# VIS4ROB-lab/covins

Hardware: AMD Instinct MI355X
Metric: GBA iterations/sec, 5-agent EuRoC merged map (higher is better)
Workload: dtype f64

## Files before the change

covins_amd/backend.py:

```python
from __future__ import annotations

import ctypes as C
import os
import subprocess
from typing import Optional, Tuple

import numpy as np

from . import capi
from .capi import FlatProblem, Options, Result, dptr, iptr

_HERE = os.path.dirname(os.path.abspath(__file__))
_SO = os.path.join(_HERE, "libcovgpu.so")
if os.environ.get("COVGPU_LIBRARY"):
    _SO = os.environ["COVGPU_LIBRARY"]
_LIB: Optional[C.CDLL] = None


class CovGpuError(RuntimeError):
    pass


def build(force: bool = False) -> str:
    args = ["make", "-C", os.path.join(_HERE, "csrc"), "-j8"]
# ... 234 lines not shown
        f = np.ascontiguousarray(f, dtype=np.float64).reshape(-1, 4, 3)
        P = np.ascontiguousarray(P, dtype=np.float64).reshape(-1, 4, 3)
        n = f.shape[0]
        T = np.zeros((max(n, 1), 4, 7)); ns = np.zeros(max(n, 1), np.int32); ch = np.zeros(max(n, 1), np.int32)
        self._check(lib().covgpu_p3p_batch(self._h, n, dptr(f), dptr(P), dptr(T), iptr(ns), iptr(ch)))
        return T[:n], ns[:n], ch[:n]

    def set_profiling(self, on: bool):
        lib().covgpu_set_profiling(self._h, int(on))

    def profile(self) -> dict:
        out = np.zeros(16)
        lib().covgpu_get_profile2(self._h, dptr(out))
        return dict(build_ms=out[0], n_build=int(out[1]), factor_ms=out[2], n_factor=int(out[3]), syrk_ms=out[4],
                    n_syrk=int(out[5]), syrk_flops=out[6], offdiag_blocks=int(out[7]),
                    potrf_ms=out[8], n_potrf=int(out[9]), potrf_flops=out[10], plan_flops=out[11])

    def layout(self) -> dict:
        out = (C.c_int64 * 16)()
        lib().covgpu_get_layout(self._h, out)
        keys = ("shard_world", "shard_rank", "top_unknowns", "top_levels", "allreduce_kib", "stream_ordering", "dense_order", "covisible_pairs",
                "edge_pairs", "chains", "device_mib", "nd_fronts", "nd_levels", "nd_serial_panels", "nd_root_order", "nd_front_mib")
        return {k: int(out[i]) for i, k in enumerate(keys)}

    def residual_norms(self, prob, opt):
        out = np.zeros(prob.O); s = prob.as_struct()
        self._check(lib().covgpu_reprojection_residual_norms(self._h, C.byref(opt), C.byref(s), dptr(out)))
        return out

    def linearize_reprojection(self, prob, opt):
        O = prob.O
# ... 55 lines not shown
```

covins_amd/csrc/common.hpp:

```cpp
#pragma once
#include <hip/hip_runtime.h>
#include <atomic>
#include <cstdlib>
#include <stdint.h>

#include <map>
#include <unordered_map>
#include <utility>
#include <vector>

#include "../../include/covgpu.h"

namespace covgpu {

constexpr int kTile = 128;

struct DevProblem {
  int K, A, L, O, I, E, S;
  int D;
  int n;
  int npad;
  int N;
  int vi;
  int lm_group;
// ... 117 lines not shown
  return P.Sred + (size_t)(6 * pi + r) * P.npad + (6 * pj + c);
}

enum { SC_COST = 0, SC_JV2 = 1, SC_GG = 2, SC_GN2 = 3, SC_GDOT = 4, SC_GMAX = 5, SC_GS = 6, SC_SN2 = 7, SC_XN2 = 8,
       SC_VV = 9, SC_VG = 10, SC_NN = 11, SC_JA = 12, SC_JB = 13, SC_JC = 14,
       SC_COUNT = 16 };

struct CholAux;
inline bool first_use_on_device(std::atomic<unsigned long long>& seen) {
  int d = 0;
  if (hipGetDevice(&d) != hipSuccess || d < 0 || d > 63) return true;
  const unsigned long long bit = 1ull << d;
  return (seen.fetch_or(bit, std::memory_order_acq_rel) & bit) == 0;
}
struct DevSignal { long long* flag = nullptr; long long seq = 0; };
inline int env_int(const char* name, int fallback) {
  const char* e = getenv(name);
  return e != nullptr ? atoi(e) : fallback;
}
void launch_kobs_build(const DevProblem& P, int* pair_oa, int* pair_ob, size_t nent, hipStream_t st);
void launch_lm_lin(const DevProblem& P, double mu, hipStream_t st, DevSignal sig = DevSignal());
void launch_lm_build(const DevProblem& P, double mu, hipStream_t st, hipEvent_t pose_system_cleared = nullptr, hipStream_t side = nullptr,
                     hipEvent_t ev_lin = nullptr, hipEvent_t ev_kf = nullptr, CholAux* ax = nullptr);
void launch_lm_backsub(const DevProblem& P, const double* dp, double* out_all, hipStream_t st);
void launch_obs_jvp(const DevProblem& P, const double* v_all, hipStream_t st);
void launch_obs_cost(const DevProblem& P, const double* pose, const double* lm, hipStream_t st);
void launch_obs_linearize(const DevProblem& P, double* r, double* Jp, double* Jl, double* cost, hipStream_t st);
void launch_obs_norms(const DevProblem& P, double* norms, hipStream_t st);
void launch_lm_outliers(const DevProblem& P, double th, unsigned char* erase, int* left, unsigned long long* counts, hipStream_t st);

// ... 58 lines not shown
  long long* gate_flags = nullptr;
  int* gate_dead = nullptr;
  int* gate_dead_h = nullptr;
  std::unordered_map<hipEvent_t, int> gate_slot;
  std::map<std::pair<hipEvent_t, hipStream_t>, int> gate_slot_es;
  std::vector<long long> gate_seq;
  long long gate_counter = 0;
  double gate_timeout_s = 3.0;
  long gate_signals = 0, gate_waits = 0;
  void record(hipEvent_t e, hipStream_t s, int tag = 0);
  void wait(hipStream_t s, hipEvent_t e0, hipEvent_t e1 = nullptr, hipEvent_t e2 = nullptr, hipEvent_t e3 = nullptr);
  DevSignal publish_handle(hipEvent_t e, hipStream_t s, int tag = 0);
  void record_handle(DevSignal d, hipStream_t s);
  void sync(hipStream_t s, hipEvent_t r0, int tag0, hipEvent_t r1, int tag1, hipEvent_t w0 = nullptr, hipEvent_t w1 = nullptr, hipEvent_t w2 = nullptr,
            hipEvent_t w3 = nullptr);
  int gate_slot_of(hipEvent_t e, hipStream_t s);
  long long* gate_log = nullptr; int gate_log_n = 0;
  std::vector<int> gate_log_tag; std::vector<char> gate_log_kind; std::vector<int> gate_tag_of_slot;
  static constexpr int kGateLogMax = 16384;
  bool gate_failed() const { return gate_dead_h != nullptr && *(volatile int*)gate_dead_h != 0; }
  void gates_disable();
};
struct BwdXfer {
  const int* gidx = nullptr;
  const int *own_g = nullptr, *st_g = nullptr, *own_dims = nullptr, *st_dims = nullptr;
  double* x = nullptr;
  int first = 0;
};
struct DenseBatch {
  int n = 0; size_t sM = 0, sL = 0, sR = 0;
// ... 37 lines not shown
void launch_bwd_front(const double* S, int tI, int ntiles, int nchunk, double* y, const double* Linv, int nbt, size_t sL, size_t sR, hipStream_t st,
                      const long long* btab, const int* live, BwdXfer xf, int* cnt, double* scr);
void launch_bwd_pipe(const double* S, int tI, int ntiles, int nchunk, double* y, const double* Linv, int nbt, size_t sL, size_t sR, hipStream_t st,
                     const long long* btab, const int* live, BwdXfer xf, double* pipe, int* dead, int* dead_h, double timeout_s);
void launch_pipe_fill(double* buf, size_t n, hipStream_t st);
constexpr int kBwdTreeMax = 8;
constexpr int kPipeChunk = 128;
struct BwdTreeLevel {
  int nbt, T, nchunk, tI, first;
  double* y; size_t bsR; const double* Dinv; size_t bsL; const long long* btab; const int* live;
  size_t scr_off, xpub_off;
};
void launch_bwd_tree(const double* M, const BwdTreeLevel* lev, int nlev, BwdXfer xf, double* pipe, int* dead, int* dead_h, double timeout_s, hipStream_t st,
                     bool form64 = false);
unsigned long long pipe_empty_word();
void launch_trsm_sub(double* S, size_t ld, int t0, int w, int r0, int r1, const double* Linv, double* b, int npad, int nbt, size_t sM, size_t sL,
                     size_t sR, const int* live, int tI, hipStream_t st, bool chain = false, const long long* btab = nullptr, int nb = -1, const int* own = nullptr);
void launch_bwd_step_sub(const double* S, size_t ld, int p, const double* Linv_p, double* y, double* x, int ncol, int nblocks, int nbt, size_t sM,
                         size_t sL, size_t sR, hipStream_t st, const long long* btab = nullptr, const int* live = nullptr, int tI = 0,
                         BwdXfer xf = BwdXfer());

struct PgoHostPlan { std::vector<std::vector<int>> block_kf; std::vector<int> border_kf; };
bool pgo_plan_analyse(int K, int E, const int* ei, const int* ej, PgoHostPlan& out);
struct PgoPlan {
  bool active = false;
  int nblk = 0, nIpad = 0, ntot = 0;
  int nb = 0;
  int* idx = nullptr;
  double *M = nullptr, *rhs = nullptr, *Linv = nullptr;
  int* idx_b = nullptr;
  double *Sb = nullptr, *rhs_b = nullptr, *Linv_b = nullptr;
};
// ... 113 lines not shown
```

covins_amd/csrc/k_chol.hip:

```cpp
#include <algorithm>
#include <cstdio>
#include <cstdlib>
#include <mutex>

#include "common.hpp"
#include "dev_math.hpp"

namespace covgpu {
using namespace covdev;

typedef double v4f64 __attribute__((ext_vector_type(4)));

#ifdef COVGPU_PROBE
__device__ long long g_probe[8];
#define PROBE(i) do { if (threadIdx.x == 0) g_probe[i] = wall_clock64(); } while (0)
#define PROBE_ACC(i, t0) do { if (threadIdx.x == 0) g_probe[i] += wall_clock64() - (t0); } while (0)
#define PROBE_T0() wall_clock64()
#else
#define PROBE(i) do {} while (0)
#define PROBE_ACC(i, t0) do {} while (0)
#define PROBE_T0() 0
#endif

constexpr int KC = 16;
// ... 175 lines not shown
      }
    __syncthreads();
    if (tid < TSA) {
      double t = 0.0;
#pragma unroll
      for (int w2 = 0; w2 < WGC; ++w2) t += sp[w2 * TSA + tid];
      g.rhs[(size_t)batch * g.bsR + g.ra0 + ti * kTile + qr * TSA + tid] -= t;
    }
  }
}

template <int MODE>
__global__ __launch_bounds__(256, 2) void k_gemm_abt(GemmArgs g) { gemm_abt_body<MODE, kTile, kTile, KC, PFF>(g); }
template <int MODE, int TSA, int TSB>
__global__ __launch_bounds__(256, 2) void k_gemm_abt_q(GemmArgs g) { gemm_abt_body<MODE, TSA, TSB, KCQ, (MODE == MODE_SYRK_RECT ? PFR : PFQ)>(g); }

static hipStream_t make_side_stream(int priority) {
  hipStream_t s2 = nullptr;
  (void)hipStreamCreateWithPriority(&s2, hipStreamNonBlocking, priority);
  return s2;
}

void CholAux::init() {
  int lo = 0, hi = 0;
  (void)hipDeviceGetStreamPriorityRange(&lo, &hi);
  if (!head) (void)hipStreamCreateWithPriority(&head, hipStreamNonBlocking, hi);
  if (!mid) mid = make_side_stream(hi);
  if (!aux) aux = make_side_stream(lo);
  if (!ev_zero) (void)hipEventCreateWithFlags(&ev_zero, hipEventDisableTiming);
  if (!ev_lin) (void)hipEventCreateWithFlags(&ev_lin, hipEventDisableTiming);
  if (!ev_kf) (void)hipEventCreateWithFlags(&ev_kf, hipEventDisableTiming);
  if (!ev_fill) (void)hipEventCreateWithFlags(&ev_fill, hipEventDisableTiming);
  if (!ev_xb) (void)hipEventCreateWithFlags(&ev_xb, hipEventDisableTiming);
  if (!ev_xa) (void)hipEventCreateWithFlags(&ev_xa, hipEventDisableTiming);
  if (!bwd_cnt && hipMalloc((void**)&bwd_cnt, 65536 * sizeof(int)) == hipSuccess) (void)hipMemset(bwd_cnt, 0, 65536 * sizeof(int));
  if (!gate_dead && hipMalloc((void**)&gate_dead, sizeof(int)) == hipSuccess) (void)hipMemset(gate_dead, 0, sizeof(int));
  if (!gate_dead_h && hipHostMalloc((void**)&gate_dead_h, 4 * sizeof(int), hipHostMallocDefault) == hipSuccess) gate_dead_h[0] = gate_dead_h[1] = gate_dead_h[2] = gate_dead_h[3] = 0;
  if (const char* e = getenv("COVGPU_GATE_TIMEOUT_S")) gate_timeout_s = std::max(getenv("COVGPU_GATE_TIMEOUT_MIN") ? atof(getenv("COVGPU_GATE_TIMEOUT_MIN")) : 0.01, atof(e));
  if (!gate_flags && !gates_broken) {
    static const bool want = env_int("COVGPU_GATES", 1) != 0;
    if (want && gate_dead != nullptr && gate_dead_h != nullptr && hipMalloc((void**)&gate_flags, kGateSlots * sizeof(long long)) == hipSuccess) {
      (void)hipMemset(gate_flags, 0, kGateSlots * sizeof(long long));
      (void)hipDeviceSynchronize();
      gates_on = true;
      if (getenv("COVGPU_GATE_LOG") && hipMalloc((void**)&gate_log, 2 * (size_t)kGateLogMax * sizeof(long long)) != hipSuccess) gate_log = nullptr;
    } else gates_broken = true;
  }
}
__global__ void k_signal(long long* flag, long long seq, long long* log) {
  if (threadIdx.x == 0) {
    __hip_atomic_store(flag, seq, __ATOMIC_RELAXED, __HIP_MEMORY_SCOPE_AGENT);
    if (log) log[0] = wall_clock64();
  }
}
__global__ void k_signal2(DevSignal a, DevSignal b) {
  if (threadIdx.x != 0) return;
// ... 36 lines not shown
    if ((int)gate_seq.size() <= slot) gate_seq.resize(slot + 1, 0);
  }
  gate_slot[e] = slot;
  return slot;
}
void CholAux::record(hipEvent_t e, hipStream_t s, int tag) {
  if (!gates_on) { (void)hipEventRecord(e, s); return; }
  const int slot = gate_slot_of(e, s);
  if (slot < 0) { gate_slot.erase(e); (void)hipEventRecord(e, s); return; }
  gate_seq[slot] = ++gate_counter;
  long long* lg = nullptr;
  if ((int)gate_tag_of_slot.size() <= slot) gate_tag_of_slot.resize(slot + 1, 0);
  gate_tag_of_slot[slot] = tag;
  if (gate_log != nullptr && gate_log_n < kGateLogMax) { lg = gate_log + 2 * (size_t)gate_log_n++; gate_log_tag.push_back(tag); gate_log_kind.push_back('S'); }
  hipLaunchKernelGGL(k_signal, dim3(1), dim3(64), 0, s, gate_flags + slot, gate_seq[slot], lg);
  ++gate_signals;
}
DevSignal CholAux::publish_handle(hipEvent_t e, hipStream_t s, int tag) {
  DevSignal d;
  if (!gates_on) return d;
  const int slot = gate_slot_of(e, s);
  if (slot < 0) { gate_slot.erase(e); return d; }
  gate_seq[slot] = ++gate_counter;
  if ((int)gate_tag_of_slot.size() <= slot) gate_tag_of_slot.resize(slot + 1, 0);
  gate_tag_of_slot[slot] = tag;
  d.flag = gate_flags + slot; d.seq = gate_seq[slot];
  ++gate_signals;
  return d;
}
void CholAux::record_handle(DevSignal d, hipStream_t s) { if (d.flag != nullptr) hipLaunchKernelGGL(k_signal2, dim3(1), dim3(64), 0, s, d, DevSignal()); }
void CholAux::wait(hipStream_t s, hipEvent_t e0, hipEvent_t e1, hipEvent_t e2, hipEvent_t e3) { sync(s, nullptr, 0, nullptr, 0, e0, e1, e2, e3); }
void CholAux::sync(hipStream_t s, hipEvent_t r0, int tag0, hipEvent_t r1, int tag1, hipEvent_t e0, hipEvent_t e1, hipEvent_t e2, hipEvent_t e3) {
  hipEvent_t es[4] = {e0, e1, e2, e3};
  if (!gates_on) {
    if (r0 != nullptr) record(r0, s, tag0);
    if (r1 != nullptr) record(r1, s, tag1);
    for (hipEvent_t e : es) if (e != nullptr) (void)hipStreamWaitEvent(s, e, 0);
    return;
  }
  GateArgs g; g.n = 0; g.dead = gate_dead; g.dead_h = gate_dead_h; g.limit = (long long)(gate_timeout_s * 1e8); g.log = nullptr; g.np = 0; g.base = gate_flags;
  g.pf[0] = g.pf[1] = nullptr; g.ps[0] = g.ps[1] = 0;
  {
    hipEvent_t rs[2] = {r0, r1}; const int tags[2] = {tag0, tag1};
    for (int i = 0; i < 2; ++i) {
      if (rs[i] == nullptr) continue;
// ... 7 lines not shown
  }
  int first_tag = g.np > 0 ? -(r0 != nullptr ? tag0 : tag1) : 0;
  for (hipEvent_t e : es) {
    if (e == nullptr) continue;
    auto it = gate_slot.find(e);
    if (it == gate_slot.end()) { (void)hipStreamWaitEvent(s, e, 0); continue; }
    if (gate_seq[it->second] == 0) continue;
    if (g.n == 0 && g.np == 0 && it->second < (int)gate_tag_of_slot.size()) first_tag = gate_tag_of_slot[it->second];
    g.f[g.n] = gate_flags + it->second; g.s[g.n] = gate_seq[it->second]; ++g.n;
  }
  if (g.n == 0 && g.np == 0) return;
  if (gate_log != nullptr && gate_log_n < kGateLogMax) { g.log = gate_log + 2 * (size_t)gate_log_n++; gate_log_tag.push_back(first_tag); gate_log_kind.push_back('G'); }
  for (int i = g.n; i < 4; ++i) { g.f[i] = nullptr; g.s[i] = 0; }
  hipLaunchKernelGGL(k_gate, dim3(1), dim3(64), 0, s, g);
  ++gate_waits;
}
void CholAux::gates_disable() {
  gates_on = false; gates_broken = true;
  pipe_broken = true;
  if (bwd_pipe) { launch_pipe_fill(bwd_pipe, bwd_pipe_elems, nullptr); (void)hipDeviceSynchronize(); }
  gate_slot.clear(); gate_slot_es.clear(); gate_seq.clear();
  if (gate_dead) (void)hipMemset(gate_dead, 0, sizeof(int));
  if (gate_dead_h) *gate_dead_h = 0;
}
void CholAux::TriCache::clear() {
  for (int* p : list) if (p) (void)hipFree(p);
  for (int* p : listC) if (p) (void)hipFree(p);
  listC.clear(); countC.clear();
  if (listA) (void)hipFree(listA);
  if (listB) (void)hipFree(listB);
// ... 10 lines not shown
  if (head) { (void)hipStreamDestroy(head); head = nullptr; }
  for (auto e : ev) (void)hipEventDestroy(e);
  for (auto e : prof_ev) (void)hipEventDestroy(e);
  for (auto e : prof_ev2) (void)hipEventDestroy(e);
  prof_ev2.clear();
  for (auto e : panel_ev) (void)hipEventDestroy(e);
  panel_ev.clear();
  ev.clear(); prof_ev.clear();
  if (ev_zero) { (void)hipEventDestroy(ev_zero); ev_zero = nullptr; }
  if (ev_lin) { (void)hipEventDestroy(ev_lin); ev_lin = nullptr; }
  if (ev_kf) { (void)hipEventDestroy(ev_kf); ev_kf = nullptr; }
  if (ev_fill) { (void)hipEventDestroy(ev_fill); ev_fill = nullptr; }
  if (ev_xb) { (void)hipEventDestroy(ev_xb); ev_xb = nullptr; }
  if (ev_xa) { (void)hipEventDestroy(ev_xa); ev_xa = nullptr; }
  if (bwd_cnt) { (void)hipFree(bwd_cnt); bwd_cnt = nullptr; }
  if (gate_flags) { (void)hipFree(gate_flags); gate_flags = nullptr; }
  if (gate_dead) { (void)hipFree(gate_dead); gate_dead = nullptr; }
  if (gate_log) { (void)hipFree(gate_log); gate_log = nullptr; }
  if (gate_dead_h) { (void)hipHostFree(gate_dead_h); gate_dead_h = nullptr; }
  gates_on = false; gate_slot.clear(); gate_slot_es.clear(); gate_seq.clear();
  if (bwd_scr) { (void)hipFree(bwd_scr); bwd_scr = nullptr; bwd_scr_elems = 0; }
  if (bwd_pipe) { (void)hipFree(bwd_pipe); bwd_pipe = nullptr; bwd_pipe_elems = 0; }
  if (aux) { (void)hipStreamDestroy(aux); aux = nullptr; }
}
void CholAux::mark(hipStream_t s, int tag) {
  static const bool trace_panels = getenv("COVGPU_TRACE_PANELS") != nullptr;
  if (!trace_panels) return;
  while ((int)panel_ev.size() <= panel_n) { hipEvent_t e; (void)hipEventCreate(&e); panel_ev.push_back(e); }
  if ((int)panel_tag.size() <= panel_n) panel_tag.resize(panel_n + 1);
  (void)hipEventRecord(panel_ev[panel_n], s);
// ... 25 lines not shown
  if (!profile) return;
  for (size_t i = 0; i < prof_flops.size(); ++i) {
    float ms = 0;
    if (hipEventElapsedTime(&ms, prof_ev[2 * i], prof_ev[2 * i + 1]) != hipSuccess) continue;
    syrk_ms += ms; syrk_flops += prof_flops[i]; n_syrk++;
  }
  prof_flops.clear();
  for (size_t i = 0; i < prof_flops2.size(); ++i) {
    float ms = 0;
    if (hipEventElapsedTime(&ms, prof_ev2[2 * i], prof_ev2[2 * i + 1]) != hipSuccess) continue;
    potrf_ms += ms; potrf_flops += prof_flops2[i]; n_potrf++;
  }
  prof_flops2.clear();
}

static const int kQuarterMax = env_int("COVGPU_QUARTER_MAX", 1024);
constexpr int kRectQuarterMax = 512;

void dense_cholesky_solve_raw(double* S, double* b, double* Linv, int* flag, int npad, hipStream_t st, CholAux& ax, int tstop, bool solve,
                              DenseBatch bt) {
  const int nbt = bt.n > 0 ? bt.n : 1;
  const int T = npad / kTile;
  const size_t ld = (size_t)npad;
  const size_t lds_gemm = (size_t)2 * kTile * LDT * sizeof(double);
  static std::atomic<unsigned long long> attr_seen{0};
  if (first_use_on_device(attr_seen)) {
    (void)hipFuncSetAttribute(reinterpret_cast<const void*>(k_gemm_abt<MODE_SYRK_TRI>), hipFuncAttributeMaxDynamicSharedMemorySize, (int)lds_gemm);
    (void)hipFuncSetAttribute(reinterpret_cast<const void*>(k_gemm_abt<MODE_SYRK_RECT>), hipFuncAttributeMaxDynamicSharedMemorySize, (int)lds_gemm);
  }
  ax.init();
  const int NP = (T + 1) / 2;
  while ((int)ax.ev.size() < 9 * (NP + 1)) { hipEvent_t e; (void)hipEventCreateWithFlags(&e, hipEventDisableTiming); ax.ev.push_back(e); }
  if (ax.profile) while (ax.prof_ev.size() < 2 * (ax.prof_flops.size() + (size_t)NP + 1)) { hipEvent_t e; (void)hipEventCreate(&e); ax.prof_ev.push_back(e); }
  hipEvent_t* eH = ax.ev.data();
  hipEvent_t* eB = eH + (NP + 1);
  hipEvent_t* eC = eB + (NP + 1);
  hipEvent_t* e1 = eC + (NP + 1);
  hipEvent_t* e2 = e1 + (NP + 1);
  hipEvent_t* e3 = e2 + (NP + 1);
  hipEvent_t* eRc = e3 + (NP + 1);
  hipEvent_t* eHp = eRc + (NP + 1);
  hipEvent_t* eA = eHp + (NP + 1);

  auto rect = [&](int r0, int r1, int tc0, int ntc, int kt0, int KD, hipStream_t s2, bool quad) {
    if (r1 <= r0 || ntc <= 0 || KD <= 0) return;
    GemmArgs g{S, ld, kt0 * kTile, KD, r0 * kTile, tc0 * kTile, tc0 * kTile, r1 - r0, nullptr, nullptr, nullptr, bt.sM, bt.sL, bt.sR, bt.live, bt.tI, nullptr, bt.tab, bt.own_dims};
    if (quad) hipLaunchKernelGGL((k_gemm_abt_q<MODE_SYRK_RECT, 64, 64>), dim3(ntc, r1 - r0, 4 * nbt), dim3(256), (size_t)(64 + 64) * (KCQ + kLdsPad) * sizeof(double), s2, g);
    else hipLaunchKernelGGL(k_gemm_abt<MODE_SYRK_RECT>, dim3(ntc, r1 - r0, nbt), dim3(256), lds_gemm, s2, g);
  };

  hipStream_t M = st, H = ax.head, R = ax.mid, B = ax.aux;
  auto wait = [&ax](hipStream_t s2, hipEvent_t e0, hipEvent_t e1 = nullptr, hipEvent_t e2 = nullptr, hipEvent_t e3 = nullptr) { ax.wait(s2, e0, e1, e2, e3); };
  auto record = [&ax](hipEvent_t e, hipStream_t s2, int tag = 0) { ax.record(e, s2, tag); };
  const int Pstop = (tstop >= 0 && tstop < T) ? tstop / 2 : NP;
  auto kd = [&](int Pp) {
    const int full = std::min(2, T - 2 * Pp) * kTile;
    if (bt.own_max <= 0) return full;
    return std::max(0, std::min(full, ((bt.own_max - 2 * Pp * kTile + 31) / 32) * 32));
  };
  auto kd_front = [&](int Pp, int a, int chunk) {
    if (bt.own_dims_h == nullptr) return kd(Pp);
    const int real = bt.own_dims_h[a] - 2 * Pp * kTile;
    return real <= 0 ? 0 : std::min(kd(Pp), ((real + chunk - 1) / chunk) * chunk);
  };
  if (bt.tri_slot >= (int)ax.tri_lev.size()) ax.tri_lev.resize(bt.tri_slot + 1);
  CholAux::TriCache& tc = bt.tri_slot >= 0 ? ax.tri_lev[bt.tri_slot] : ax.tri0;
  auto build_list = [&](int t0, int tb, int part, int*& d_out, int& n_out) {
    d_out = nullptr; n_out = 0;
// ... 86 lines not shown
      record(eB[P], B, 100 * (P + 1) + 11);
      record(eA[P], B, 100 * (P + 1) + 18);
      Plast = P;
      break;
    }
    ax.mark(M, P);
    if (Pstop < NP && P == Pstop - 1) {
      const int nbp = bt.own_max > 0 ? std::max(0, std::min(8 * w, (bt.own_max - t0 * kTile + 15) / 16)) : -1;
      potrf(t0, w, nbp);
      if (trace2) ax.mark(M, 100 * (P + 1) + 1);
      if (P == 0 && bt.pre_trsm != nullptr) wait(M, bt.pre_trsm);
      bool split_done = false;
      if (T > h0) {
        const bool split = bt.split_ta > 0 && bt.live_h != nullptr && kd(P) > 0 && (tc.listA != nullptr || tc.listB != nullptr);
        const bool waitedA = split && P >= 1;
        if (P > 0) wait(M, h1 > h0 ? eHp[P] : nullptr, T > h1 ? e2[P] : nullptr, waitedA ? eA[P - 1] : nullptr);
        launch_trsm_sub(S, ld, t0, w, h0, T, Linv, b, npad, nbt, bt.sM, bt.sL, bt.sR, bt.live, bt.tI, M, true, bt.tab, nbp, bt.own_dims);
        if (split) { record(eH[P], M, 100 * (P + 1) + 10); wait(B, eH[P]); }
        if (P >= 1 && !waitedA) wait(M, eB[P - 1]);
        const int tb = h0, nt = T - tb;
        auto syrk = [&](hipStream_t s2, const int* list, int count, double flops) {
          GemmArgs g{S, ld, t0 * kTile, kd(P), tb * kTile, tb * kTile, tb * kTile, nt, nullptr, nullptr, nullptr, bt.sM, bt.sL, bt.sR, bt.live, bt.tI, nullptr, bt.tab, bt.own_dims};
          g.tri = list; g.beta0_off = bt.beta0_off; g.beta0 = bt.beta0;
          if (ax.profile) (void)hipEventRecord(ax.prof_ev[2 * ax.prof_flops.size()], s2);
          if (list != nullptr && count <= kQuarterMax)
            hipLaunchKernelGGL((k_gemm_abt_q<MODE_SYRK_TRI, 64, 64>), dim3(count, 1, 4), dim3(256), (size_t)(64 + 64) * (KCQ + kLdsPad) * sizeof(double), s2, g);
          else if (list != nullptr) hipLaunchKernelGGL(k_gemm_abt<MODE_SYRK_TRI>, dim3(count, 1), dim3(256), lds_gemm, s2, g);
          else {
            const int Ts = (nt + 7) / 8, ns = Ts * (Ts + 1) / 2, nblk = ((ns + 7) / 8) * 8 * 64;
            hipLaunchKernelGGL(k_gemm_abt<MODE_SYRK_TRI>, dim3(nblk, nbt), dim3(256), lds_gemm, s2, g);
          }
          if (ax.profile) {
// ... 29 lines not shown
      Plast = P; split_last = split_done; tail_on_chain = true;
      break;
    }
    bool bulk_wait_rc = false;
    {
      const int nbp = bt.own_max > 0 ? std::max(0, std::min(8 * w, (bt.own_max - t0 * kTile + 15) / 16)) : -1;
      const double bulk_pairs = (T - (t0 + 4) > 0) ? 0.5 * (double)(T - (t0 + 4)) * (T - (t0 + 4) + 1) * nbt : 0.0;
      static const double chain_pairs = getenv("COVGPU_CHAIN_PAIRS") ? atof(getenv("COVGPU_CHAIN_PAIRS")) : 0.0;
      const bool chain_bound = bulk_pairs <= chain_pairs;
      potrf(t0, w, nbp);
      if (P == 0 && bt.pre_trsm != nullptr) wait(M, bt.pre_trsm);
      bool waitedA = false;
      hipEvent_t rec1 = !chain_bound ? e1[P] : nullptr;
      if (h1 > h0) {
        waitedA = P >= 1 && P + 1 < NP;
        ax.sync(M, rec1, 100 * (P + 1) + 13, nullptr, 0, P > 0 ? eHp[P] : nullptr, waitedA ? eA[P - 1] : nullptr);
        rec1 = nullptr;
        launch_trsm_sub(S, ld, t0, w, h0, h1, Linv, b, npad, nbt, bt.sM, bt.sL, bt.sR, bt.live, bt.tI, M, true, bt.tab, nbp, bt.own_dims);
        if (trace2) ax.mark(M, 100 * (P + 1) + 2);
      }
      if (rec1 != nullptr) record(rec1, M, 100 * (P + 1) + 13);
      const bool eh_now = !chain_bound && P + 1 == NP;
      if (eh_now) record(eH[P], M, 100 * (P + 1) + 10);
      if (P + 1 < NP) {
        const int u0 = t0 + 2, uw = (T - u0 >= 2) ? 2 : 1;
        if (P >= 1 && !waitedA) wait(M, eA[P - 1]);
        rect(u0, u0 + uw, u0, uw, t0, kd(P), M, true);
        if (trace2) ax.mark(M, 100 * (P + 1) + 3);
      }
      if (chain_bound || eh_now) record(chain_bound ? eH[P] : eRc[P], M, 100 * (P + 1) + (chain_bound ? 10 : 16));
      else ax.sync(M, eH[P], 100 * (P + 1) + 10, eRc[P], 100 * (P + 1) + 16);
      if (T > h1) {
        wait(R, chain_bound ? eH[P] : e1[P]);
        launch_trsm_sub(S, ld, t0, w, h1, T, Linv, b, npad, nbt, bt.sM, bt.sL, bt.sR, bt.live, bt.tI, R, false, bt.tab, nbp, bt.own_dims);
        if (trace2) ax.mark(R, 100 * (P + 1) + 4);
      }
      record(eC[P], R, 100 * (P + 1) + 12);
      bulk_wait_rc = !chain_bound;
    }
    const int tb = t0 + 4, nt = T - tb;
    bool recA = false;
    wait(B, eC[P], bulk_wait_rc ? eRc[P] : nullptr);
    if (nt > 0 && kd(P) > 0) {
      const int Ts = (nt + 7) / 8, ns = Ts * (Ts + 1) / 2, nblk = ((ns + 7) / 8) * 8 * 64;
      GemmArgs g{S, ld, t0 * kTile, kd(P), tb * kTile, tb * kTile, tb * kTile, nt, nullptr, nullptr, nullptr, bt.sM, bt.sL, bt.sR, bt.live, bt.tI, nullptr, bt.tab, bt.own_dims};
      const bool listed = bt.live_h != nullptr && P < (int)tc.list.size() && tc.list[P] != nullptr;
// ... 113 lines not shown
```

covins_amd/csrc/k_panel.hip:

```cpp
#include <cstdio>
#include <cstdlib>

#include <algorithm>

#include "common.hpp"
#include "dev_math.hpp"

namespace covgpu {

typedef double v4f64 __attribute__((ext_vector_type(4)));

#ifdef COVGPU_PROBE
__device__ long long g_pprobe[8];
__device__ long long g_pstep[4][16];
#define PSTEP(k, j, t0) do { if ((threadIdx.x & 63) == 0) g_pstep[k][j] = clock64() - (t0); } while (0)
__device__ long long g_parr[16][16];
#define PARR(j, t0) do { if ((threadIdx.x & 63) == 0) g_parr[threadIdx.x >> 6][j] = clock64() - (t0); } while (0)
#ifndef PPROBE_WAVE
#define PPROBE_WAVE 1
#endif
#define PPROBE_DECL() long long pacc[8] = {0, 0, 0, 0, 0, 0, 0, 0}
#define PPROBE_ACC(i, t0) do { pacc[i] += clock64() - (t0); } while (0)
#define PPROBE_T0() clock64()
#define PPROBE_FLUSH() do { if (threadIdx.x == 0) for (int i_ = 1; i_ < 6; ++i_) g_pprobe[i_] = pacc[i_]; if (threadIdx.x == 64 * PPROBE_WAVE) { g_pprobe[6] = pacc[6]; g_pprobe[7] = pacc[7]; } } while (0)
// ... 458 lines not shown
#pragma unroll
    for (int m = 0; m < MB; ++m) {
      const v4f64 y4 = *reinterpret_cast<const v4f64*>(yv + PB * (4 * m + wave));
#pragma unroll
      for (int s = 0; s < 4; ++s) part += acc[m][s] * y4[s];
    }
    part += __shfl_xor(part, 16, 64);
    part += __shfl_xor(part, 32, 64);
    if (fk == 0) spart[wave][n] = part;
    lds_barrier();
    if (wave == 0 && fk == 0) g.rhs[(size_t)batch * g.bsR + row0 + n] -= ((spart[0][n] + spart[1][n]) + spart[2][n]) + spart[3][n];
  }
}

template <int NB>
__global__ __launch_bounds__(256) void k_trsm_sub4(TrsmSubArgs g) {
  __shared__ v4f64 zall[16][64];
  __shared__ double spart[4][16];
  __shared__ int zcount;
  if (g.live != nullptr) {
    const int batch = blockIdx.y, row0 = g.r0 + PB * (int)blockIdx.x;
    const int nI = g.live[2 * batch], nO = g.live[2 * batch + 1];
    const int tp = g.k0 / kTile, tr = row0 / kTile;
    if (!(tp < nI || (tp >= g.tI && tp - g.tI < nO))) return;
    if (!(tr < nI || (tr >= g.tI && tr - g.tI < nO))) return;
  }
  int nbf = NB;
  if (g.own != nullptr) {
    const int real = g.own[blockIdx.y] - g.k0;
    if (real <= 0) return;
    nbf = (real + PB - 1) / PB;
  }
  if (threadIdx.x == 0) zcount = 0;
  __syncthreads();
  if (NB > 4 && nbf <= 4) { trsm_sub4_body<4>(g, zall, &zcount, spart); return; }
  if (NB > 8 && nbf <= 8) { trsm_sub4_body<8>(g, zall, &zcount, spart); return; }
  if (NB > 12 && nbf <= 12) { trsm_sub4_body<12>(g, zall, &zcount, spart); return; }
  trsm_sub4_body<NB>(g, zall, &zcount, spart);
}


__global__ __launch_bounds__(256) void k_bwd_step_sub(const double* __restrict__ M, size_t ld, int p, const double* __restrict__ Dinv,
                                                       double* __restrict__ y, double* __restrict__ x, int ncol, size_t bsM, size_t bsL, size_t bsR,
                                                       const long long* __restrict__ btab, const int* __restrict__ live, int tI, BwdXfer xf) {
  if (live != nullptr) {
    const int nI = live[2 * blockIdx.y], nO = live[2 * blockIdx.y + 1];
    if (!(p < nI || (p >= tI && p - tI < nO))) return;
  }
  if (btab != nullptr) { M += (size_t)btab[2 * blockIdx.y]; ld = (size_t)btab[2 * blockIdx.y + 1]; }
  else M += (size_t)blockIdx.y * bsM;
  y += (size_t)blockIdx.y * bsR; x += (size_t)blockIdx.y * bsR;
  if (Dinv != nullptr) Dinv += (size_t)blockIdx.y * bsL;
  __shared__ double sx[kTile];
// ... 682 lines not shown
  }
  double* Lp = Linv + (size_t)t0 * kTile * kTile;
  const double* yb = b ? b + npad : nullptr;
  if (list == nullptr) {
    hipLaunchKernelGGL(k_potrf_panel, dim3(nbt), dim3(64 * NW), kPanelLds, st, S, ld, t0 * kTile, nb, Lp, flag, (const double*)b, (double*)yb, sM, sL, sR, btab, own, list);
    return;
  }
  constexpr int kSmallMin = 384;
  if (n_small <= kSmallMin) { n_big += n_small; n_small = 0; }
  if (n_big > 0) hipLaunchKernelGGL(k_potrf_panel, dim3(n_big), dim3(64 * NW), kPanelLds, st, S, ld, t0 * kTile, nb, Lp, flag, (const double*)b, (double*)yb, sM, sL, sR, btab, own, list);
  if (n_small > 0)
    hipLaunchKernelGGL(k_potrf_panel4, dim3(n_small), dim3(256), kPanelLds4, st, S, ld, t0 * kTile, std::min(nb, 8), Lp, flag, (const double*)b, (double*)yb, sM, sL, sR, btab, own,
                       list + n_big);
}

void launch_trsm_sub(double* S, size_t ld, int t0, int w, int r0, int r1, const double* Linv, double* b, int npad, int nbt, size_t sM, size_t sL,
                     size_t sR, const int* live, int tI, hipStream_t st, bool chain, const long long* btab, int nb, const int* own) {
  if (r1 <= r0 || nb == 0) return;
  TrsmSubArgs g{S, ld, t0 * kTile, r0 * kTile, Linv + (size_t)t0 * kTile * kTile, b, b ? b + npad : nullptr, sM, sL, sR, live, tI, chain ? 1 : 0, btab, own};
  const dim3 grid((r1 - r0) * (kTile / PB), nbt);
  const int need = nb > 0 ? std::min(nb, 8 * w) : 8 * w;
  if (need <= 4) hipLaunchKernelGGL(k_trsm_sub4<4>, grid, dim3(256), 0, st, g);
  else if (need <= 8) hipLaunchKernelGGL(k_trsm_sub4<8>, grid, dim3(256), 0, st, g);
  else if (need <= 12) hipLaunchKernelGGL(k_trsm_sub4<12>, grid, dim3(256), 0, st, g);
  else hipLaunchKernelGGL(k_trsm_sub4<16>, grid, dim3(256), 0, st, g);
}

void launch_bwd_front(const double* S, int tI, int ntiles, int nchunk, double* y, const double* Linv, int nbt, size_t sL, size_t sR, hipStream_t st,
                      const long long* btab, const int* live, BwdXfer xf, int* cnt, double* scr) {
  hipLaunchKernelGGL(k_bwd_front, dim3(ntiles * nchunk, nbt), dim3(256), 0, st, S, tI, nchunk, y, Linv, sL, sR, btab, live, xf, cnt, scr);
}

void launch_bwd_step_sub(const double* S, size_t ld, int p, const double* Linv_p, double* y, double* x, int ncol, int nblocks, int nbt, size_t sM,
                         size_t sL, size_t sR, hipStream_t st, const long long* btab, const int* live, int tI, BwdXfer xf) {
  hipLaunchKernelGGL(k_bwd_step_sub, dim3(nblocks, nbt), dim3(256), 0, st, S, ld, p, Linv_p, y, x, ncol, sM, sL, sR, btab, live, tI, xf);
}

}
```

covins_amd/csrc/solver.hip:

```cpp
#include <dlfcn.h>

#include <algorithm>
#include <atomic>
#include <chrono>
#include <condition_variable>
#include <memory>
#include <mutex>
#include <cmath>
#include <cstdio>
#include <cstdlib>
#include <cstring>
#include <string>
#include <thread>
#include <vector>

#include "common.hpp"
#include "nd_plan.hpp"

using namespace covgpu;

static thread_local std::string g_err;
extern "C" const char* covgpu_last_error(void) { return g_err.c_str(); }

#define HIPCHK(expr)                                                                            \
// ... 323 lines not shown
}

extern "C" void covgpu_set_profiling(covgpu_context* c, int on) {
  c->profiling = on; c->prof = covgpu_profile_t();
  c->chol.profile = on != 0; c->chol.syrk_ms = 0; c->chol.syrk_flops = 0; c->chol.n_syrk = 0;
  c->chol.potrf_ms = 0; c->chol.potrf_flops = 0; c->chol.n_potrf = 0;
}
extern "C" void covgpu_get_profile(covgpu_context* c, double* out) {
  out[0] = c->prof.t_build_ms; out[1] = (double)c->prof.n_build; out[2] = c->prof.t_factor_ms; out[3] = (double)c->prof.n_factor;
  out[4] = c->chol.syrk_ms; out[5] = (double)c->chol.n_syrk; out[6] = c->chol.syrk_flops;
  out[7] = (double)(c->have ? c->P.npairs + c->P.nepairs : 0);
}
extern "C" void covgpu_get_profile2(covgpu_context* c, double* out) {
  covgpu_get_profile(c, out);
  out[8] = c->chol.potrf_ms; out[9] = (double)c->chol.n_potrf; out[10] = c->chol.potrf_flops; out[11] = c->have ? c->nd.plan_flops : 0.0;
  out[12] = out[13] = out[14] = out[15] = 0.0;
}

extern "C" void covgpu_get_layout(covgpu_context* c, int64_t* out) {
  for (int i = 0; i < 16; ++i) out[i] = 0;
  if (!c->have) return;
  const DevProblem& P = c->P;
  out[0] = c->sharded ? c->world : 0; out[1] = c->sharded ? c->rank : 0; out[2] = c->nd.ntop;
  out[3] = (int64_t)c->nd.lev.size() - c->nd.top_lev0;
  out[4] = c->nd.dist ? (int64_t)((c->nd.dist_solve_elems * sizeof(double)) >> 10)
                      : (int64_t)(((size_t)c->nd.n_top_tiles * kTile * kTile + c->nd.rhs_top + 2 * (size_t)c->nd.ntop) * sizeof(double)) >> 10;
  out[5] = c->chol.pipe_broken ? -1 : c->chol.gates_on ? 1 : 0;
  out[6] = P.npad; out[7] = P.npairs; out[8] = P.nepairs; out[9] = P.nchains; out[10] = (int64_t)(c->alloc_bytes >> 20);
  if (P.nd) {
    out[11] = P.nd_nnodes; out[12] = P.nd_nlev;
    for (const NdLevel& L : c->nd.lev) out[13] += L.nI / 256;
// ... 1697 lines not shown
```

Before: 291.1.

## Fold gate wait/signal kernels into trsm and rect-syrk kernel prologues/epilogues

Replaces the separate one-block gate and signal kernels launched before and after small trsm_sub and rect-syrk launches on the main chain stream with a ChainSync struct. Kernels now spin on the flags in their prologue and publish completion through a last-block ticket in their epilogue. The aim is to cut per-panel kernel launch count and the latency of the extra tiny kernels on the critical Cholesky path. Folding applies only to grids of up to 256 workgroups, because every block of a folded kernel spins. This risks deadlock or occupancy waste, which the timeout guards against, and adds gate-launch counters to the profile output.

```diff
diff --git a/covins_amd/backend.py b/covins_amd/backend.py
--- a/covins_amd/backend.py
+++ b/covins_amd/backend.py
@@ -272,7 +272,8 @@
         lib().covgpu_get_profile2(self._h, dptr(out))
         return dict(build_ms=out[0], n_build=int(out[1]), factor_ms=out[2], n_factor=int(out[3]), syrk_ms=out[4],
                     n_syrk=int(out[5]), syrk_flops=out[6], offdiag_blocks=int(out[7]),
-                    potrf_ms=out[8], n_potrf=int(out[9]), potrf_flops=out[10], plan_flops=out[11])
+                    potrf_ms=out[8], n_potrf=int(out[9]), potrf_flops=out[10], plan_flops=out[11],
+                    gate_launches=int(out[12]), signal_launches=int(out[13]), gate_folds=int(out[14]))
 
     def layout(self) -> dict:
         out = (C.c_int64 * 16)()
diff --git a/covins_amd/csrc/common.hpp b/covins_amd/csrc/common.hpp
--- a/covins_amd/csrc/common.hpp
+++ b/covins_amd/csrc/common.hpp
@@ -155,6 +155,64 @@
   return (seen.fetch_or(bit, std::memory_order_acq_rel) & bit) == 0;
 }
 struct DevSignal { long long* flag = nullptr; long long seq = 0; };
+struct ChainSync {
+  const long long* wf[4]; long long ws[4]; int nw;
+  long long* pf[2]; long long ps[2]; int np;
+  int at_start;
+  int* ticket;
+  int* dead; int* dead_h; long long limit; const long long* base;
+  long long* wlog; long long* plog;
+  hipEvent_t rev[2];
+};
+#if defined(__HIPCC__)
+__device__ inline bool chain_wait(const ChainSync& c) {
+  const bool pub0 = c.at_start != 0 && c.np > 0;
+  if (c.nw == 0 && !pub0) return true;
+  __shared__ int s_go;
+  if (threadIdx.x == 0) {
+    const bool first = blockIdx.x == 0 && blockIdx.y == 0 && blockIdx.z == 0;
+    if (pub0 && first) {
+      for (int i = 0; i < c.np; ++i) __hip_atomic_store(c.pf[i], c.ps[i], __ATOMIC_RELAXED, __HIP_MEMORY_SCOPE_AGENT);
+      if (c.plog != nullptr) c.plog[0] = wall_clock64();
+    }
+    int go = 1;
+    const long long t0 = wall_clock64();
+    for (int i = 0; i < c.nw && go; ++i) {
+      unsigned spins = 0;
+      while (__hip_atomic_load(c.wf[i], __ATOMIC_RELAXED, __HIP_MEMORY_SCOPE_AGENT) < c.ws[i]) {
+        __builtin_amdgcn_s_sleep(1);
+        if ((++spins & 127u) == 0) {
+          if (__hip_atomic_load(c.dead, __ATOMIC_RELAXED, __HIP_MEMORY_SCOPE_AGENT) != 0) { go = 0; break; }
+          if (wall_clock64() - t0 > c.limit) {
+            __hip_atomic_store(c.dead, 1, __ATOMIC_RELAXED, __HIP_MEMORY_SCOPE_AGENT);
+            __hip_atomic_store(c.dead_h + 1, (int)(c.wf[i] - c.base), __ATOMIC_RELAXED, __HIP_MEMORY_SCOPE_SYSTEM);
+            __hip_atomic_store(c.dead_h + 2, (int)c.ws[i], __ATOMIC_RELAXED, __HIP_MEMORY_SCOPE_SYSTEM);
+            __hip_atomic_store(c.dead_h + 3, (int)__hip_atomic_load(c.wf[i], __ATOMIC_RELAXED, __HIP_MEMORY_SCOPE_AGENT), __ATOMIC_RELAXED, __HIP_MEMORY_SCOPE_SYSTEM);
+            __hip_atomic_store(c.dead_h, 1, __ATOMIC_RELEASE, __HIP_MEMORY_SCOPE_SYSTEM);
+            go = 0; break;
+          }
+        }
+      }
+    }
+    if (c.nw > 0) __builtin_amdgcn_fence(__ATOMIC_ACQUIRE, "agent");
+    if (c.wlog != nullptr && first && c.nw > 0) { c.wlog[0] = t0; c.wlog[1] = wall_clock64(); }
+    s_go = go;
+  }
+  __syncthreads();
+  return s_go != 0;
+}
+__device__ inline void chain_publish(const ChainSync& c) {
+  if (c.np == 0 || c.at_start != 0) return;
+  __syncthreads();
+  if (threadIdx.x != 0) return;
+  __builtin_amdgcn_fence(__ATOMIC_RELEASE, "agent");
+  const int blocks = (int)(gridDim.x * gridDim.y * gridDim.z);
+  if (__hip_atomic_fetch_add(c.ticket, 1, __ATOMIC_ACQ_REL, __HIP_MEMORY_SCOPE_AGENT) != blocks - 1) return;
+  __hip_atomic_store(c.ticket, 0, __ATOMIC_RELAXED, __HIP_MEMORY_SCOPE_AGENT);
+  for (int i = 0; i < c.np; ++i) __hip_atomic_store(c.pf[i], c.ps[i], __ATOMIC_RELEASE, __HIP_MEMORY_SCOPE_AGENT);
+  if (c.plog != nullptr) c.plog[0] = wall_clock64();
+}
+#endif
 inline int env_int(const char* name, int fallback) {
   const char* e = getenv(name);
   return e != nullptr ? atoi(e) : fallback;
@@ -243,6 +301,12 @@
   void record_handle(DevSignal d, hipStream_t s);
   void sync(hipStream_t s, hipEvent_t r0, int tag0, hipEvent_t r1, int tag1, hipEvent_t w0 = nullptr, hipEvent_t w1 = nullptr, hipEvent_t w2 = nullptr,
             hipEvent_t w3 = nullptr);
+  ChainSync fold(hipStream_t s, bool at_start, hipEvent_t r0, int tag0, hipEvent_t r1, int tag1, hipEvent_t w0 = nullptr, hipEvent_t w1 = nullptr,
+                 hipEvent_t w2 = nullptr, hipEvent_t w3 = nullptr);
+  void unfold(const ChainSync& c, hipStream_t s);
+  void land(const ChainSync& c, hipStream_t s);
+  int* gate_ticket = nullptr;
+  long gate_signal_launches = 0, gate_folds = 0;
   int gate_slot_of(hipEvent_t e, hipStream_t s);
   long long* gate_log = nullptr; int gate_log_n = 0;
   std::vector<int> gate_log_tag; std::vector<char> gate_log_kind; std::vector<int> gate_tag_of_slot;
@@ -310,8 +374,9 @@
 void launch_bwd_tree(const double* M, const BwdTreeLevel* lev, int nlev, BwdXfer xf, double* pipe, int* dead, int* dead_h, double timeout_s, hipStream_t st,
                      bool form64 = false);
 unsigned long long pipe_empty_word();
-void launch_trsm_sub(double* S, size_t ld, int t0, int w, int r0, int r1, const double* Linv, double* b, int npad, int nbt, size_t sM, size_t sL,
-                     size_t sR, const int* live, int tI, hipStream_t st, bool chain = false, const long long* btab = nullptr, int nb = -1, const int* own = nullptr);
+bool launch_trsm_sub(double* S, size_t ld, int t0, int w, int r0, int r1, const double* Linv, double* b, int npad, int nbt, size_t sM, size_t sL,
+                     size_t sR, const int* live, int tI, hipStream_t st, bool chain = false, const long long* btab = nullptr, int nb = -1, const int* own = nullptr,
+                     const ChainSync* cs = nullptr);
 void launch_bwd_step_sub(const double* S, size_t ld, int p, const double* Linv_p, double* y, double* x, int ncol, int nblocks, int nbt, size_t sM,
                          size_t sL, size_t sR, hipStream_t st, const long long* btab = nullptr, const int* live = nullptr, int tI = 0,
                          BwdXfer xf = BwdXfer());
diff --git a/covins_amd/csrc/k_chol.hip b/covins_amd/csrc/k_chol.hip
--- a/covins_amd/csrc/k_chol.hip
+++ b/covins_amd/csrc/k_chol.hip
@@ -213,6 +213,11 @@
 __global__ __launch_bounds__(256, 2) void k_gemm_abt(GemmArgs g) { gemm_abt_body<MODE, kTile, kTile, KC, PFF>(g); }
 template <int MODE, int TSA, int TSB>
 __global__ __launch_bounds__(256, 2) void k_gemm_abt_q(GemmArgs g) { gemm_abt_body<MODE, TSA, TSB, KCQ, (MODE == MODE_SYRK_RECT ? PFR : PFQ)>(g); }
+template <int MODE, int TSA, int TSB>
+__global__ __launch_bounds__(256, 2) void k_gemm_abt_qc(GemmArgs g, ChainSync cs) {
+  if (chain_wait(cs)) gemm_abt_body<MODE, TSA, TSB, KCQ, (MODE == MODE_SYRK_RECT ? PFR : PFQ)>(g);
+  chain_publish(cs);
+}
 
 static hipStream_t make_side_stream(int priority) {
   hipStream_t s2 = nullptr;
@@ -233,12 +238,13 @@
   if (!ev_xb) (void)hipEventCreateWithFlags(&ev_xb, hipEventDisableTiming);
   if (!ev_xa) (void)hipEventCreateWithFlags(&ev_xa, hipEventDisableTiming);
   if (!bwd_cnt && hipMalloc((void**)&bwd_cnt, 65536 * sizeof(int)) == hipSuccess) (void)hipMemset(bwd_cnt, 0, 65536 * sizeof(int));
+  if (!gate_ticket && hipMalloc((void**)&gate_ticket, kGateSlots * sizeof(int)) == hipSuccess) (void)hipMemset(gate_ticket, 0, kGateSlots * sizeof(int));
   if (!gate_dead && hipMalloc((void**)&gate_dead, sizeof(int)) == hipSuccess) (void)hipMemset(gate_dead, 0, sizeof(int));
   if (!gate_dead_h && hipHostMalloc((void**)&gate_dead_h, 4 * sizeof(int), hipHostMallocDefault) == hipSuccess) gate_dead_h[0] = gate_dead_h[1] = gate_dead_h[2] = gate_dead_h[3] = 0;
   if (const char* e = getenv("COVGPU_GATE_TIMEOUT_S")) gate_timeout_s = std::max(getenv("COVGPU_GATE_TIMEOUT_MIN") ? atof(getenv("COVGPU_GATE_TIMEOUT_MIN")) : 0.01, atof(e));
   if (!gate_flags && !gates_broken) {
     static const bool want = env_int("COVGPU_GATES", 1) != 0;
-    if (want && gate_dead != nullptr && gate_dead_h != nullptr && hipMalloc((void**)&gate_flags, kGateSlots * sizeof(long long)) == hipSuccess) {
+    if (want && gate_dead != nullptr && gate_dead_h != nullptr && gate_ticket != nullptr && hipMalloc((void**)&gate_flags, kGateSlots * sizeof(long long)) == hipSuccess) {
       (void)hipMemset(gate_flags, 0, kGateSlots * sizeof(long long));
       (void)hipDeviceSynchronize();
       gates_on = true;
@@ -305,7 +311,7 @@
   gate_tag_of_slot[slot] = tag;
   if (gate_log != nullptr && gate_log_n < kGateLogMax) { lg = gate_log + 2 * (size_t)gate_log_n++; gate_log_tag.push_back(tag); gate_log_kind.push_back('S'); }
   hipLaunchKernelGGL(k_signal, dim3(1), dim3(64), 0, s, gate_flags + slot, gate_seq[slot], lg);
-  ++gate_signals;
+  ++gate_signals; ++gate_signal_launches;
 }
 DevSignal CholAux::publish_handle(hipEvent_t e, hipStream_t s, int tag) {
   DevSignal d;
@@ -319,7 +325,11 @@
   ++gate_signals;
   return d;
 }
-void CholAux::record_handle(DevSignal d, hipStream_t s) { if (d.flag != nullptr) hipLaunchKernelGGL(k_signal2, dim3(1), dim3(64), 0, s, d, DevSignal()); }
+void CholAux::record_handle(DevSignal d, hipStream_t s) {
+  if (d.flag == nullptr) return;
+  hipLaunchKernelGGL(k_signal2, dim3(1), dim3(64), 0, s, d, DevSignal());
+  ++gate_signal_launches;
+}
 void CholAux::wait(hipStream_t s, hipEvent_t e0, hipEvent_t e1, hipEvent_t e2, hipEvent_t e3) { sync(s, nullptr, 0, nullptr, 0, e0, e1, e2, e3); }
 void CholAux::sync(hipStream_t s, hipEvent_t r0, int tag0, hipEvent_t r1, int tag1, hipEvent_t e0, hipEvent_t e1, hipEvent_t e2, hipEvent_t e3) {
   hipEvent_t es[4] = {e0, e1, e2, e3};
@@ -357,6 +367,74 @@
   for (int i = g.n; i < 4; ++i) { g.f[i] = nullptr; g.s[i] = 0; }
   hipLaunchKernelGGL(k_gate, dim3(1), dim3(64), 0, s, g);
   ++gate_waits;
+}
+__global__ void k_chain_gate(ChainSync cs) {
+  (void)chain_wait(cs);
+  chain_publish(cs);
+}
+ChainSync CholAux::fold(hipStream_t s, bool at_start, hipEvent_t r0, int tag0, hipEvent_t r1, int tag1, hipEvent_t w0, hipEvent_t w1, hipEvent_t w2,
+                        hipEvent_t w3) {
+  ChainSync c{};
+  hipEvent_t ws[4] = {w0, w1, w2, w3};
+  c.at_start = at_start ? 1 : 0;
+  if (!gates_on) {
+    if (at_start) { if (r0 != nullptr) (void)hipEventRecord(r0, s); if (r1 != nullptr) (void)hipEventRecord(r1, s); }
+    for (hipEvent_t e : ws) if (e != nullptr) (void)hipStreamWaitEvent(s, e, 0);
+    if (!at_start) { c.rev[0] = r0; c.rev[1] = r1; }
+    return c;
+  }
+  if (at_start) {
+    hipEvent_t rs[2] = {r0, r1}; const int tags[2] = {tag0, tag1};
+    for (int i = 0; i < 2; ++i) {
+      if (rs[i] == nullptr) continue;
+      const int slot = gate_slot_of(rs[i], s);
+      if (slot < 0) { gate_slot.erase(rs[i]); (void)hipEventRecord(rs[i], s); continue; }
+      gate_seq[slot] = ++gate_counter;
+      if ((int)gate_tag_of_slot.size() <= slot) gate_tag_of_slot.resize(slot + 1, 0);
+      gate_tag_of_slot[slot] = tags[i];
+      if (c.np == 0 && gate_log != nullptr && gate_log_n < kGateLogMax) { c.plog = gate_log + 2 * (size_t)gate_log_n++; gate_log_tag.push_back(tags[i]); gate_log_kind.push_back('S'); }
+      c.pf[c.np] = gate_flags + slot; c.ps[c.np] = gate_seq[slot]; ++c.np; ++gate_signals;
+    }
+    r0 = r1 = nullptr;
+  }
+  c.dead = gate_dead; c.dead_h = gate_dead_h; c.limit = (long long)(gate_timeout_s * 1e8); c.base = gate_flags;
+  int first_tag = 0;
+  for (hipEvent_t e : ws) {
+    if (e == nullptr) continue;
+    auto it = gate_slot.find(e);
+    if (it == gate_slot.end()) { (void)hipStreamWaitEvent(s, e, 0); continue; }
+    if (gate_seq[it->second] == 0) continue;
+    if (c.nw == 0 && it->second < (int)gate_tag_of_slot.size()) first_tag = gate_tag_of_slot[it->second];
+    c.wf[c.nw] = gate_flags + it->second; c.ws[c.nw] = gate_seq[it->second]; ++c.nw;
+  }
+  if (c.nw > 0 && gate_log != nullptr && gate_log_n < kGateLogMax) {
+    c.wlog = gate_log + 2 * (size_t)gate_log_n++; gate_log_tag.push_back(first_tag); gate_log_kind.push_back('G');
+  }
+  hipEvent_t rs[2] = {r0, r1}; const int tags[2] = {tag0, tag1};
+  for (int i = 0; i < 2; ++i) {
+    if (rs[i] == nullptr) continue;
+    const int slot = gate_slot_of(rs[i], s);
+    if (slot < 0) { gate_slot.erase(rs[i]); c.rev[i] = rs[i]; continue; }
+    gate_seq[slot] = ++gate_counter;
+    if ((int)gate_tag_of_slot.size() <= slot) gate_tag_of_slot.resize(slot + 1, 0);
+    gate_tag_of_slot[slot] = tags[i];
+    if (c.np == 0) {
+      c.ticket = gate_ticket + slot;
+      if (gate_log != nullptr && gate_log_n < kGateLogMax) { c.plog = gate_log + 2 * (size_t)gate_log_n++; gate_log_tag.push_back(tags[i]); gate_log_kind.push_back('S'); }
+    }
+    c.pf[c.np] = gate_flags + slot; c.ps[c.np] = gate_seq[slot]; ++c.np; ++gate_signals;
+  }
+  if (c.nw > 0 || c.np > 0) ++gate_folds;
+  return c;
+}
+void CholAux::unfold(const ChainSync& c, hipStream_t s) {
+  if (c.nw == 0 && c.np == 0) return;
+  hipLaunchKernelGGL(k_chain_gate, dim3(1), dim3(64), 0, s, c);
+  if (c.nw > 0) ++gate_waits; else ++gate_signal_launches;
+  --gate_folds;
+}
+void CholAux::land(const ChainSync& c, hipStream_t s) {
+  for (hipEvent_t e : c.rev) if (e != nullptr) (void)hipEventRecord(e, s);
 }
 void CholAux::gates_disable() {
   gates_on = false; gates_broken = true;
@@ -397,6 +475,7 @@
   if (ev_xb) { (void)hipEventDestroy(ev_xb); ev_xb = nullptr; }
   if (ev_xa) { (void)hipEventDestroy(ev_xa); ev_xa = nullptr; }
   if (bwd_cnt) { (void)hipFree(bwd_cnt); bwd_cnt = nullptr; }
+  if (gate_ticket) { (void)hipFree(gate_ticket); gate_ticket = nullptr; }
   if (gate_flags) { (void)hipFree(gate_flags); gate_flags = nullptr; }
   if (gate_dead) { (void)hipFree(gate_dead); gate_dead = nullptr; }
   if (gate_log) { (void)hipFree(gate_log); gate_log = nullptr; }
@@ -452,6 +531,7 @@
   prof_flops2.clear();
 }
 
+constexpr long kFoldMaxWg = 256;
 static const int kQuarterMax = env_int("COVGPU_QUARTER_MAX", 1024);
 constexpr int kRectQuarterMax = 512;
 
@@ -480,16 +560,27 @@
   hipEvent_t* eHp = eRc + (NP + 1);
   hipEvent_t* eA = eHp + (NP + 1);
 
-  auto rect = [&](int r0, int r1, int tc0, int ntc, int kt0, int KD, hipStream_t s2, bool quad) {
-    if (r1 <= r0 || ntc <= 0 || KD <= 0) return;
+  auto rect = [&](int r0, int r1, int tc0, int ntc, int kt0, int KD, hipStream_t s2, bool quad, const ChainSync* cs = nullptr) {
+    if (r1 <= r0 || ntc <= 0 || KD <= 0) return false;
     GemmArgs g{S, ld, kt0 * kTile, KD, r0 * kTile, tc0 * kTile, tc0 * kTile, r1 - r0, nullptr, nullptr, nullptr, bt.sM, bt.sL, bt.sR, bt.live, bt.tI, nullptr, bt.tab, bt.own_dims};
-    if (quad) hipLaunchKernelGGL((k_gemm_abt_q<MODE_SYRK_RECT, 64, 64>), dim3(ntc, r1 - r0, 4 * nbt), dim3(256), (size_t)(64 + 64) * (KCQ + kLdsPad) * sizeof(double), s2, g);
+    if (cs != nullptr) hipLaunchKernelGGL((k_gemm_abt_qc<MODE_SYRK_RECT, 64, 64>), dim3(ntc, r1 - r0, 4 * nbt), dim3(256), (size_t)(64 + 64) * (KCQ + kLdsPad) * sizeof(double), s2, g, *cs);
+    else if (quad) hipLaunchKernelGGL((k_gemm_abt_q<MODE_SYRK_RECT, 64, 64>), dim3(ntc, r1 - r0, 4 * nbt), dim3(256), (size_t)(64 + 64) * (KCQ + kLdsPad) * sizeof(double), s2, g);
     else hipLaunchKernelGGL(k_gemm_abt<MODE_SYRK_RECT>, dim3(ntc, r1 - r0, nbt), dim3(256), lds_gemm, s2, g);
+    return true;
   };
 
   hipStream_t M = st, H = ax.head, R = ax.mid, B = ax.aux;
   auto wait = [&ax](hipStream_t s2, hipEvent_t e0, hipEvent_t e1 = nullptr, hipEvent_t e2 = nullptr, hipEvent_t e3 = nullptr) { ax.wait(s2, e0, e1, e2, e3); };
   auto record = [&ax](hipEvent_t e, hipStream_t s2, int tag = 0) { ax.record(e, s2, tag); };
+  auto fold = [&ax, M](long wgs, bool at_start, hipEvent_t r0, int tag0, hipEvent_t r1, int tag1, hipEvent_t w0 = nullptr, hipEvent_t w1 = nullptr,
+                       hipEvent_t w2 = nullptr) {
+    if (wgs > kFoldMaxWg) {
+      if (at_start) { ax.sync(M, r0, tag0, r1, tag1, w0, w1, w2); return ChainSync{}; }
+      ax.wait(M, w0, w1, w2); w0 = w1 = w2 = nullptr;
+    }
+    return ax.fold(M, at_start, r0, tag0, r1, tag1, w0, w1, w2);
+  };
+  auto carried = [&ax, M](const ChainSync& cs, bool launched) { if (!launched) ax.unfold(cs, M); ax.land(cs, M); };
   const int Pstop = (tstop >= 0 && tstop < T) ? tstop / 2 : NP;
   auto kd = [&](int Pp) {
     const int full = std::min(2, T - 2 * Pp) * kTile;
@@ -606,8 +697,9 @@
       if (T > h0) {
         const bool split = bt.split_ta > 0 && bt.live_h != nullptr && kd(P) > 0 && (tc.listA != nullptr || tc.listB != nullptr);
         const bool waitedA = split && P >= 1;
-        if (P > 0) wait(M, h1 > h0 ? eHp[P] : nullptr, T > h1 ? e2[P] : nullptr, waitedA ? eA[P - 1] : nullptr);
-        launch_trsm_sub(S, ld, t0, w, h0, T, Linv, b, npad, nbt, bt.sM, bt.sL, bt.sR, bt.live, bt.tI, M, true, bt.tab, nbp, bt.own_dims);
+        const ChainSync cs = P > 0 ? fold((long)(T - h0) * (kTile / 16) * nbt, false, nullptr, 0, nullptr, 0, h1 > h0 ? eHp[P] : nullptr,
+                                          T > h1 ? e2[P] : nullptr, waitedA ? eA[P - 1] : nullptr) : ChainSync{};
+        carried(cs, launch_trsm_sub(S, ld, t0, w, h0, T, Linv, b, npad, nbt, bt.sM, bt.sL, bt.sR, bt.live, bt.tI, M, true, bt.tab, nbp, bt.own_dims, &cs));
         if (split) { record(eH[P], M, 100 * (P + 1) + 10); wait(B, eH[P]); }
         if (P >= 1 && !waitedA) wait(M, eB[P - 1]);
         const int tb = h0, nt = T - tb;
@@ -667,22 +759,24 @@
       hipEvent_t rec1 = !chain_bound ? e1[P] : nullptr;
       if (h1 > h0) {
         waitedA = P >= 1 && P + 1 < NP;
-        ax.sync(M, rec1, 100 * (P + 1) + 13, nullptr, 0, P > 0 ? eHp[P] : nullptr, waitedA ? eA[P - 1] : nullptr);
+        const ChainSync cs = fold((long)(h1 - h0) * (kTile / 16) * nbt, true, rec1, 100 * (P + 1) + 13, nullptr, 0, P > 0 ? eHp[P] : nullptr,
+                                  waitedA ? eA[P - 1] : nullptr);
         rec1 = nullptr;
-        launch_trsm_sub(S, ld, t0, w, h0, h1, Linv, b, npad, nbt, bt.sM, bt.sL, bt.sR, bt.live, bt.tI, M, true, bt.tab, nbp, bt.own_dims);
+        carried(cs, launch_trsm_sub(S, ld, t0, w, h0, h1, Linv, b, npad, nbt, bt.sM, bt.sL, bt.sR, bt.live, bt.tI, M, true, bt.tab, nbp, bt.own_dims, &cs));
         if (trace2) ax.mark(M, 100 * (P + 1) + 2);
       }
       if (rec1 != nullptr) record(rec1, M, 100 * (P + 1) + 13);
       const bool eh_now = !chain_bound && P + 1 == NP;
       if (eh_now) record(eH[P], M, 100 * (P + 1) + 10);
+      hipEvent_t ra = chain_bound ? eH[P] : eh_now ? eRc[P] : eH[P], rb = (chain_bound || eh_now) ? nullptr : eRc[P];
+      const int taga = 100 * (P + 1) + ((chain_bound || !eh_now) ? 10 : 16), tagb = 100 * (P + 1) + 16;
       if (P + 1 < NP) {
         const int u0 = t0 + 2, uw = (T - u0 >= 2) ? 2 : 1;
-        if (P >= 1 && !waitedA) wait(M, eA[P - 1]);
-        rect(u0, u0 + uw, u0, uw, t0, kd(P), M, true);
+        const ChainSync cs = fold((long)uw * uw * 4 * nbt, false, ra, taga, rb, tagb, P >= 1 && !waitedA ? eA[P - 1] : nullptr);
+        carried(cs, rect(u0, u0 + uw, u0, uw, t0, kd(P), M, true, &cs));
         if (trace2) ax.mark(M, 100 * (P + 1) + 3);
-      }
-      if (chain_bound || eh_now) record(chain_bound ? eH[P] : eRc[P], M, 100 * (P + 1) + (chain_bound ? 10 : 16));
-      else ax.sync(M, eH[P], 100 * (P + 1) + 10, eRc[P], 100 * (P + 1) + 16);
+      } else if (rb == nullptr) record(ra, M, taga);
+      else ax.sync(M, ra, taga, rb, tagb);
       if (T > h1) {
         wait(R, chain_bound ? eH[P] : e1[P]);
         launch_trsm_sub(S, ld, t0, w, h1, T, Linv, b, npad, nbt, bt.sM, bt.sL, bt.sR, bt.live, bt.tI, R, false, bt.tab, nbp, bt.own_dims);
diff --git a/covins_amd/csrc/k_panel.hip b/covins_amd/csrc/k_panel.hip
--- a/covins_amd/csrc/k_panel.hip
+++ b/covins_amd/csrc/k_panel.hip
@@ -496,7 +496,7 @@
 }
 
 template <int NB>
-__global__ __launch_bounds__(256) void k_trsm_sub4(TrsmSubArgs g) {
+__device__ __forceinline__ void trsm_sub4_entry(const TrsmSubArgs& g) {
   __shared__ v4f64 zall[16][64];
   __shared__ double spart[4][16];
   __shared__ int zcount;
@@ -519,6 +519,11 @@
   if (NB > 8 && nbf <= 8) { trsm_sub4_body<8>(g, zall, &zcount, spart); return; }
   if (NB > 12 && nbf <= 12) { trsm_sub4_body<12>(g, zall, &zcount, spart); return; }
   trsm_sub4_body<NB>(g, zall, &zcount, spart);
+}
+template <int NB>
+__global__ __launch_bounds__(256) void k_trsm_sub4(TrsmSubArgs g, ChainSync cs) {
+  if (chain_wait(cs)) trsm_sub4_entry<NB>(g);
+  chain_publish(cs);
 }
 
 
@@ -1231,16 +1236,18 @@
                        list + n_big);
 }
 
-void launch_trsm_sub(double* S, size_t ld, int t0, int w, int r0, int r1, const double* Linv, double* b, int npad, int nbt, size_t sM, size_t sL,
-                     size_t sR, const int* live, int tI, hipStream_t st, bool chain, const long long* btab, int nb, const int* own) {
-  if (r1 <= r0 || nb == 0) return;
+bool launch_trsm_sub(double* S, size_t ld, int t0, int w, int r0, int r1, const double* Linv, double* b, int npad, int nbt, size_t sM, size_t sL,
+                     size_t sR, const int* live, int tI, hipStream_t st, bool chain, const long long* btab, int nb, const int* own, const ChainSync* cs) {
+  if (r1 <= r0 || nb == 0) return false;
+  const ChainSync c = cs != nullptr ? *cs : ChainSync{};
   TrsmSubArgs g{S, ld, t0 * kTile, r0 * kTile, Linv + (size_t)t0 * kTile * kTile, b, b ? b + npad : nullptr, sM, sL, sR, live, tI, chain ? 1 : 0, btab, own};
   const dim3 grid((r1 - r0) * (kTile / PB), nbt);
   const int need = nb > 0 ? std::min(nb, 8 * w) : 8 * w;
-  if (need <= 4) hipLaunchKernelGGL(k_trsm_sub4<4>, grid, dim3(256), 0, st, g);
-  else if (need <= 8) hipLaunchKernelGGL(k_trsm_sub4<8>, grid, dim3(256), 0, st, g);
-  else if (need <= 12) hipLaunchKernelGGL(k_trsm_sub4<12>, grid, dim3(256), 0, st, g);
-  else hipLaunchKernelGGL(k_trsm_sub4<16>, grid, dim3(256), 0, st, g);
+  if (need <= 4) hipLaunchKernelGGL(k_trsm_sub4<4>, grid, dim3(256), 0, st, g, c);
+  else if (need <= 8) hipLaunchKernelGGL(k_trsm_sub4<8>, grid, dim3(256), 0, st, g, c);
+  else if (need <= 12) hipLaunchKernelGGL(k_trsm_sub4<12>, grid, dim3(256), 0, st, g, c);
+  else hipLaunchKernelGGL(k_trsm_sub4<16>, grid, dim3(256), 0, st, g, c);
+  return true;
 }
 
 void launch_bwd_front(const double* S, int tI, int ntiles, int nchunk, double* y, const double* Linv, int nbt, size_t sL, size_t sR, hipStream_t st,
diff --git a/covins_amd/csrc/solver.hip b/covins_amd/csrc/solver.hip
--- a/covins_amd/csrc/solver.hip
+++ b/covins_amd/csrc/solver.hip
@@ -361,7 +361,7 @@
 extern "C" void covgpu_get_profile2(covgpu_context* c, double* out) {
   covgpu_get_profile(c, out);
   out[8] = c->chol.potrf_ms; out[9] = (double)c->chol.n_potrf; out[10] = c->chol.potrf_flops; out[11] = c->have ? c->nd.plan_flops : 0.0;
-  out[12] = out[13] = out[14] = out[15] = 0.0;
+  out[12] = (double)c->chol.gate_waits; out[13] = (double)c->chol.gate_signal_launches; out[14] = (double)c->chol.gate_folds; out[15] = 0.0;
 }
 
 extern "C" void covgpu_get_layout(covgpu_context* c, int64_t* out) {
```

Result: no change. 292.1, median of 6 (+0.3%).
